# pavel-paulau/query

Hardware: AMD Instinct MI355X
Metric: rows/sec filter+group-by on 100M synthetic JSON docs; achieved HBM GB/s (higher is better)
Workload: dtype int64/f64 tagged scalars (u8 tag + 8 B payload), u32 dictionary codes; 1 GPU; config2: SELECT cat, SUM(price) FROM default WHERE price > 50 GROUP BY cat @ 100000000 rows, K_cat=1000, columns resident in HBM; rows_per_gpu=100000000, groups=1000, rows_selected=49401294, agg_mode=2, spec_kernel=1

## Files before the change

### query_amd/csrc/n1k_kernels.h

```cpp
#pragma once
#include <hip/hip_runtime.h>
#include <vector>
#include "n1k_types.h"

namespace n1k {

constexpr int kFilterStreamTile = 8192;

struct OutValue {
    uint64_t tag;
    uint64_t payload;
};

struct OutPartial {
    int64_t count;
    int64_t isum;
    double fsum;
    uint32_t flags;
    uint32_t ext_tag;
    uint64_t ext_payload;
    int64_t distinct;
};

struct SynthArgs {
    uint64_t seed, first_row, nrows, total_rows;
    uint32_t k_cat, pad;
    const double* cat_cdf;
    uint32_t* cat_codes;
    uint8_t* price_tags;
    uint64_t* price_payload;
    uint8_t* user_tags;
    uint64_t* user_payload;
    uint8_t* region_tags;
    uint64_t* region_payload;
};

hipError_t launch_init_table(const Program& P, const GlobalTable& G, uint64_t first, uint64_t count,
                             unsigned long long* counters, hipStream_t st);
hipError_t launch_restamp_ranks(const Program& P, const GlobalTable& G, hipStream_t st);
hipError_t launch_rehash(const Program& P, const GlobalTable& oldt, const GlobalTable& newt, uint32_t* err_flags,
                         unsigned long long* ngroups_scratch, hipStream_t st);
hipError_t launch_scan_group(const Program& P, const ScanArgs& A, const GlobalTable& G, unsigned long long* ngroups,
                             uint32_t grid, uint32_t block, uint32_t rows_per_lane, bool direct, hipStream_t st);
hipError_t launch_scan_fast(const Program& P, const FastArgs& F, const GlobalTable& G, unsigned long long* ngroups,
                            uint32_t grid, uint32_t block, uint32_t rows_per_lane, hipStream_t st);
hipError_t launch_merge_slabs(const Program& P, const FastArgs& F, const GlobalTable& G, uint32_t nblocks,
                              unsigned long long* ngroups, hipStream_t st, uint32_t ychunks_opt = 0);
hipError_t launch_finalize_region(const Program& P, const uint64_t* region, uint64_t cap, uint64_t count, OutValue* out_keys,
                                  OutValue* out_aggs, OutPartial* out_parts, uint64_t* out_rep, uint32_t* err_flags, hipStream_t st,
                                  const uint32_t* cand = nullptr, OutValue* ord = nullptr, bool ord_is_key = false, uint32_t ord_index = 0,
                                  uint64_t* images = nullptr, bool desc = false);
hipError_t launch_add_counter(unsigned long long* p, unsigned long long v, hipStream_t st);
hipError_t launch_probe_keys(const Program& P, uint64_t nrows, const GlobalTable& G, uint32_t* err_flags, unsigned long long* ngroups,
                             uint32_t grid, hipStream_t st);
hipError_t launch_project_records(const Program& P, const ProjectArgs& A, uint32_t grid, hipStream_t st);
hipError_t launch_agg_bins(const Program& P, const BinAggArgs& A, const GlobalTable& G, unsigned long long* ngroups, uint32_t grid,
                           hipStream_t st);
size_t topk_state_bytes();
size_t topk_ncand_offset();
hipError_t launch_topk_select(const Program& P, const OutValue* vals, uint32_t stride, uint32_t index, uint64_t n, bool desc,
                              uint64_t keep, uint64_t* images, void* state, uint32_t* cand, hipStream_t st, bool sampled = false, bool images_done = false);
bool topk_can_sample(uint64_t n, uint64_t keep);
uint64_t topk_cand_entries(uint64_t n);
hipError_t launch_topk_compact(const uint32_t* cand, uint64_t ncand, uint32_t nk, uint32_t na, const OutValue* keys,
                               const OutValue* aggs, const OutPartial* parts, const uint64_t* rep, OutValue* okeys, OutValue* oaggs,
                               OutPartial* oparts, uint64_t* orep, hipStream_t st);
hipError_t launch_distinct_layout(const Program& P, const GlobalTable& G, const DistinctArgs& D, hipStream_t st);
hipError_t launch_radix_pass(const RadixArgs& A, uint32_t slices, hipStream_t st, bool have_hist = false);
hipError_t launch_distinct_dedupe(const Program& P, const GlobalTable& G, const DedupeArgs& D, uint32_t grid, uint32_t block, hipStream_t st);
size_t distinct_dedupe_lds(const DedupeArgs& D);
hipError_t launch_compact_regions(const uint64_t* region, uint32_t nreg, uint64_t cap, const unsigned long long* count, const uint64_t* off,
                                  uint64_t* dst, hipStream_t st);
hipError_t launch_regrow_regions(const uint64_t* src, uint32_t nreg, uint64_t src_cap, uint64_t* dst, uint64_t dst_cap,
                                 unsigned long long* count, hipStream_t st);
hipError_t launch_distinct_words_global(const GlobalTable& G, const uint64_t* words, uint64_t n, uint64_t* table, uint64_t mask,
                                        uint32_t key_shift, unsigned long long* counts, uint32_t* err_flags, uint32_t grid,
                                        hipStream_t st);
hipError_t launch_distinct_add_counts(const Program& P, const GlobalTable& G, const unsigned long long* counts, uint32_t glob_off,
                                      hipStream_t st, const uint32_t* veto = nullptr);
hipError_t launch_distinct_insert(const Program& P, const GlobalTable& G, const DistinctArgs& D, uint32_t* err_flags,
                                  hipStream_t st);
hipError_t launch_export_partials(const Program& P, const GlobalTable& G, uint32_t nparts, uint64_t cap, uint64_t* out,
                                  uint64_t region_words, uint32_t* err_flags, hipStream_t st);
hipError_t launch_merge_partials(const Program& P, const GlobalTable& G, uint32_t nregions, uint64_t cap, const uint64_t* in,
                                 uint64_t region_words, uint32_t* err_flags, unsigned long long* ngroups, hipStream_t st,
                                 uint64_t limit = 0, bool unique_keys = false);
hipError_t launch_arith(const ArithArgs& A, hipStream_t st);
hipError_t launch_publish_counters(const unsigned long long* src, unsigned long long* dst, uint32_t n, hipStream_t st);
hipError_t launch_partition(const Program& P, const PartArgs& A, uint32_t grid, hipStream_t st);
struct HeaderList { unsigned long long* h[kMaxParts]; };
hipError_t launch_exchange_verdict(const HeaderList& H, uint32_t nregions, uint32_t* err_flags, hipStream_t st);
hipError_t launch_stamp_verdict(unsigned long long* headers, uint32_t nregions, uint64_t stride_words, const uint32_t* err_flags,
                                uint32_t host_status, hipStream_t st);
hipError_t launch_dense_to_segments(unsigned long long* headers, uint32_t nregions, uint64_t stride_words, uint64_t sub_rows, hipStream_t st,
                                    const uint32_t* dest_cap = nullptr);
struct SpecEntry {
    const char* name;
    SpecSig sig;
    hipError_t (*launch)(const Program& P, const FastArgs& F, const GlobalTable& G, unsigned long long* ngroups,
                         uint32_t grid, uint32_t block, bool wide, const WordLogArgs& L, hipStream_t st);
// ... 48 lines not shown
```

### query_amd/csrc/n1k_kernels.hip

```cpp
#include <hip/hip_runtime.h>
#include "n1k_device.h"
#include "n1k_tables.h"
#include "n1k_scatter.h"
#include "n1k_kernels.h"
#include <algorithm>
#include <vector>

namespace n1k {


template <int R>
N1K_DEV void load_operand(const Program& P, const Operand& o, const uint64_t (&row)[R], const bool (&valid)[R],
                          uint32_t (&tag)[R], uint64_t (&pay)[R]) {
    if (o.is_const) {
#pragma unroll
        for (int j = 0; j < R; j++) {
            tag[j] = o.ctag;
            pay[j] = o.cpayload;
        }
        return;
    }
    const DevCol& c = P.cols[o.col];
    if (c.kind == COLK_DICT32) {
        const uint32_t* codes = c.codes;
// ... 1235 lines not shown
            if (!pass[j]) continue;
            uint64_t r = s_base[dest[j]] + pos[j];
            if (r >= (A.per_dest ? (uint64_t)A.dest_cap[dest[j]] : A.capacity)) {
                if (!(atomicOr(A.err_flags, (uint32_t)ERR_TABLE_FULL) & ERR_TABLE_FULL) && A.region_bytes)
                    for (uint32_t q = 0; q < A.nparts; q++)
                        atomicOr(&A.counts[(size_t)q * A.count_stride + 1], 1ull);
                pass[j] = false;
            }
            pos[j] = A.region_bytes ? r : (uint64_t)dest[j] * A.capacity + r;
        }
        __syncthreads();
        for (uint32_t d = tid; d < A.nparts; d += BLOCK) s_cnt[d] = 0;
        uint64_t roff[R];
#pragma unroll
        for (int j = 0; j < R; j++) roff[j] = A.hdr_bytes;
        for (uint32_t c = 0; c < A.ncopy; c++) {
            Operand o{};
            o.is_const = 0;
            o.col = c;
            uint32_t vt[R];
            uint64_t vp[R];
            load_operand<R>(P, o, row, pass, vt, vp);
#pragma unroll
            for (int j = 0; j < R; j++) {
                if (!pass[j]) continue;
                if (A.per_dest) {
                    char* const reg = (char*)A.counts + (size_t)dest[j] * A.region_bytes;
                    const uint64_t capd = A.dest_cap[dest[j]];
                    if (P.cols[c].kind == COLK_DICT32) {
                        ((uint32_t*)(reg + roff[j]))[pos[j]] = (uint32_t)vp[j];
                        roff[j] = part_region_next(roff[j], capd, 4);
                    } else {
                        ((uint64_t*)(reg + roff[j]))[pos[j]] = vp[j];
                        roff[j] = part_region_next(roff[j], capd, 8);
                        ((uint8_t*)(reg + roff[j]))[pos[j]] = (uint8_t)vt[j];
                        roff[j] = part_region_next(roff[j], capd, 1);
                    }
                    continue;
                }
                const size_t shift = (size_t)dest[j] * A.region_bytes;
                if (P.cols[c].kind == COLK_DICT32) {
                    ((uint32_t*)((char*)A.out_codes[c] + shift))[pos[j]] = (uint32_t)vp[j];
                } else {
                    ((uint8_t*)((char*)A.out_tags[c] + shift))[pos[j]] = (uint8_t)vt[j];
                    ((uint64_t*)((char*)A.out_payload[c] + shift))[pos[j]] = vp[j];
                }
            }
        }
    }
    if (unsupported) atomicOr(A.err_flags, (uint32_t)ERR_UNSUPPORTED_VALUE);
    if (unpackable) atomicOr(A.err_flags, (uint32_t)ERR_UNPACKABLE_KEY);
}

enum { RED_ADD_U64, RED_ADD_F64, RED_OR, RED_MIN_I64, RED_MAX_I64, RED_MIN_U64, RED_MAX_U64 };

template <int OP>
N1K_DEV uint64_t reduce_over_y(uint64_t (*red)[64], uint64_t v) {
    const uint32_t tx = threadIdx.x, ty = threadIdx.y;
    red[ty][tx] = v;
    __syncthreads();
    for (uint32_t off = 8; off > 0; off >>= 1) {
        if (ty < off) {
            uint64_t a = red[ty][tx], b = red[ty + off][tx], r;
            if (OP == RED_ADD_U64) r = a + b;
            else if (OP == RED_ADD_F64) r = f64_bits(as_f64(a) + as_f64(b));
            else if (OP == RED_OR) r = a | b;
            else if (OP == RED_MIN_I64) r = (int64_t)a < (int64_t)b ? a : b;
            else if (OP == RED_MAX_I64) r = (int64_t)a > (int64_t)b ? a : b;
            else if (OP == RED_MIN_U64) r = a < b ? a : b;
            else r = a > b ? a : b;
            red[ty][tx] = r;
        }
        __syncthreads();
    }
    uint64_t out = red[0][tx];
    __syncthreads();
    return out;
}

__global__ __launch_bounds__(1024) void merge_slabs_kernel(const Program P, const FastArgs F, const GlobalTable G,
                                                          uint32_t nblocks_total, unsigned long long* ngroups) {
    __shared__ uint64_t red[16][64];
    const uint32_t S = F.lds_slots;
    const uint32_t s = blockIdx.x * 64 + threadIdx.x;
    const bool in_range = s < S;
    if (blockIdx.x == 0 && blockIdx.y == 0 && threadIdx.y == 0) {
        unsigned long long c = 0;
        for (uint32_t b = threadIdx.x; b < nblocks_total; b += 64) c += F.block_selected[b];
        for (int off = 32; off > 0; off >>= 1) c += __shfl_down(c, off, 64);
        if (threadIdx.x == 0 && c) atomicAdd(F.rows_selected, c);
    }
    const uint32_t Y = 16 * gridDim.y, y = blockIdx.y * 16 + threadIdx.y;
    const size_t slab_words = (size_t)P.lds_words * S * Y;
    const uint32_t nblocks = (in_range && y < nblocks_total) ? (nblocks_total - y + Y - 1) / Y : 0;
    const uint64_t* base = F.slabs + (size_t)y * P.lds_words * S + (in_range ? s : 0);
    uint64_t touched = 0;
#pragma unroll 8
    for (uint32_t b = 0; b < nblocks; b++) touched |= base[b * slab_words] ^ kEmptyKey;
    touched = reduce_over_y<RED_OR>(red, touched);
    const bool leader = threadIdx.y == 0 && in_range && touched != 0;
    long long g = -1;
    if (leader) g = global_find_or_insert(G, fast_slot_key(F, s), F.err_flags, ngroups);
    uint64_t* grow = g >= 0 ? &G.acc[(size_t)g * P.glob_words] : nullptr;
    for (uint32_t a = 0; a < P.naggs; a++) {
        const AggSpec& ag = P.aggs[a];
        if (ag.distinct) continue;
        const uint64_t* l = base + (size_t)ag.lds_off * S;
        unsigned long long* w = grow ? (unsigned long long*)(grow + ag.glob_off) : nullptr;
        switch (ag.kind) {
            case AGG_COUNT:
            case AGG_COUNTN: {
                unsigned long long c = 0;
#pragma unroll 8
                for (uint32_t b = 0; b < nblocks; b++) c += l[b * slab_words];
                c = reduce_over_y<RED_ADD_U64>(red, c);
                if (w && c) atomicAdd(&w[0], c);
                break;
            }
            case AGG_SUM:
            case AGG_AVG: {
                unsigned long long lo = 0, hi = 0, fl = 0, n = 0;
                double fs = 0.0;
                const bool avg = ag.kind == AGG_AVG;
#pragma unroll 4
                for (uint32_t b = 0; b < nblocks; b++) {
                    const uint64_t* lb = l + b * slab_words;
                    int64_t x = (int64_t)lb[0];
                    double f = as_f64(lb[(size_t)S]);
                    fl |= lb[2 * (size_t)S];
                    lo += (unsigned long long)(uint32_t)x;
                    hi += (unsigned long long)(x >> 32);
                    fs += f;
                    if (avg) n += lb[3 * (size_t)S];
                }
                lo = reduce_over_y<RED_ADD_U64>(red, lo);
                hi = reduce_over_y<RED_ADD_U64>(red, hi);
                fs = as_f64(reduce_over_y<RED_ADD_F64>(red, f64_bits(fs)));
                fl = reduce_over_y<RED_OR>(red, fl);
                if (avg) n = reduce_over_y<RED_ADD_U64>(red, n);
                if (!w || !fl) break;
                if (fl & (SF_NONNEG_INT | SF_NEG_INT)) { atomicAdd(&w[0], lo); atomicAdd(&w[1], hi); }
                if (fl & SF_FLOAT) atomicAdd((double*)&w[2], fs);
                atomicOr(&w[3], fl);
                if (avg) atomicAdd(&w[4], n);
                break;
            }
            default: {
                const bool mn = ag.kind == AGG_MIN;
                unsigned long long fl = 0;
                long long iv = mn ? INT64_MAX : INT64_MIN;
                unsigned long long fv = mn ? ~0ull : 0ull, sv = mn ? ~0ull : 0ull;
#pragma unroll 4
                for (uint32_t b = 0; b < nblocks; b++) {
                    const uint64_t* lb = l + b * slab_words;
                    fl |= lb[0];
                    long long x = (long long)lb[(size_t)S];
                    unsigned long long yv = lb[2 * (size_t)S], z = lb[3 * (size_t)S];
                    iv = mn ? (x < iv ? x : iv) : (x > iv ? x : iv);
                    fv = mn ? (yv < fv ? yv : fv) : (yv > fv ? yv : fv);
                    sv = mn ? (z < sv ? z : sv) : (z > sv ? z : sv);
                }
                fl = reduce_over_y<RED_OR>(red, fl);
                if (mn) {
                    iv = (long long)reduce_over_y<RED_MIN_I64>(red, (uint64_t)iv);
                    fv = reduce_over_y<RED_MIN_U64>(red, fv);
                    sv = reduce_over_y<RED_MIN_U64>(red, sv);
                } else {
                    iv = (long long)reduce_over_y<RED_MAX_I64>(red, (uint64_t)iv);
                    fv = reduce_over_y<RED_MAX_U64>(red, fv);
                    sv = reduce_over_y<RED_MAX_U64>(red, sv);
                }
                if (!w || !fl) break;
                atomicOr(&w[0], fl);
                if (fl & MM_INT) { if (mn) atomicMin((long long*)&w[1], iv); else atomicMax((long long*)&w[1], iv); }
                if (fl & MM_FLOAT) { if (mn) atomicMin(&w[2], fv); else atomicMax(&w[2], fv); }
                if (fl & MM_STRING) { if (mn) atomicMin(&w[3], sv); else atomicMax(&w[3], sv); }
                break;
            }
        }
    }
}

__global__ void export_partials_kernel(const Program P, const GlobalTable G, uint32_t nparts, uint64_t cap,
                                       uint64_t* out, uint64_t region_words, uint32_t* err_flags) {
    uint64_t s = (uint64_t)blockIdx.x * blockDim.x + threadIdx.x;
    if (s == 0 && P.wide_count && *P.wide_count)
        for (uint32_t r = 0; r < nparts; r++) atomicOr((unsigned long long*)&out[(size_t)r * region_words + 1], 2ull);
    const uint64_t key = s < G.capacity ? G.keys[s] : kEmptyKey;
    const bool used = key != kEmptyKey;
    const uint32_t d = used ? (uint32_t)(((mix64(key) >> 32) * (uint64_t)nparts) >> 32) : 0xFFFFFFFFu;
    unsigned long long pos = 0;
    unsigned long long todo = __ballot(used);
    const uint32_t lane = threadIdx.x & 63;
    while (todo) {
        const int leader = __ffsll((long long)todo) - 1;
        const uint32_t dl = __shfl(d, leader, 64);
        const unsigned long long same = __ballot(used && d == dl);
        unsigned long long base = 0;
        if ((int)lane == leader) base = atomicAdd((unsigned long long*)&out[(size_t)dl * region_words], (unsigned long long)__popcll(same));
        base = __shfl(base, leader, 64);
        if (used && d == dl) pos = base + (unsigned long long)__popcll(same & ((1ull << lane) - 1ull));
        todo &= ~same;
    }
    if (!used) return;
    uint64_t* region = out + (size_t)d * region_words;
    if (pos >= cap) {
        if (!(atomicOr(err_flags, (uint32_t)ERR_TABLE_FULL) & ERR_TABLE_FULL))
            for (uint32_t r = 0; r < nparts; r++) atomicOr((unsigned long long*)&out[(size_t)r * region_words + 1], 1ull);
        return;
    }
    region[2 + pos] = key;
    uint64_t* acc = region + 2 + cap + pos * P.glob_words;
    for (uint32_t w = 0; w < P.glob_words; w++) acc[w] = G.acc[(size_t)s * P.glob_words + w];
}

N1K_DEV void merge_partial_record(const Program& P, const GlobalTable& G, uint64_t key, const uint64_t* l, uint32_t* err_flags,
                                  bool& fresh, bool unique_keys) {
    long long g = global_find_or_insert_quiet(G, key, err_flags, fresh);
    if (g < 0) return;
    if (fresh && unique_keys) {
        uint64_t* w = &G.acc[(size_t)g * P.glob_words];
        for (uint32_t i = 0; i < P.glob_words; i++) w[i] = l[i];
        return;
    }
    for (uint32_t a = 0; a < P.naggs; a++) {
        const AggSpec& ag = P.aggs[a];
        const uint64_t* p = l + ag.glob_off;
        unsigned long long* w = (unsigned long long*)&G.acc[(size_t)g * P.glob_words + ag.glob_off];
        if (ag.distinct) {
            atomicOr(err_flags, (uint32_t)ERR_UNSUPPORTED_VALUE);
            continue;
// ... 1160 lines not shown
    hipLaunchKernelGGL(rehash_kernel, dim3(blocks), dim3(256), 0, st, P, oldt, newt, err_flags, ngroups_scratch);
    return hipGetLastError();
}

template <int R, int BLOCK>
static hipError_t launch_scan_variant(const Program& P, const ScanArgs& A, const GlobalTable& G, unsigned long long* ngroups,
                                      uint32_t grid, bool direct, size_t shmem, hipStream_t st) {
    if (direct) {
        auto k = scan_group_kernel<R, BLOCK, true>;
        if (shmem > 48 * 1024) (void)hipFuncSetAttribute((const void*)k, hipFuncAttributeMaxDynamicSharedMemorySize, (int)shmem);
        hipLaunchKernelGGL(k, dim3(grid), dim3(BLOCK), shmem, st, P, A, G, ngroups);
    } else {
        auto k = scan_group_kernel<R, BLOCK, false>;
        if (shmem > 48 * 1024) (void)hipFuncSetAttribute((const void*)k, hipFuncAttributeMaxDynamicSharedMemorySize, (int)shmem);
        hipLaunchKernelGGL(k, dim3(grid), dim3(BLOCK), shmem, st, P, A, G, ngroups);
    }
    return hipGetLastError();
}

hipError_t launch_scan_group(const Program& P, const ScanArgs& A, const GlobalTable& G, unsigned long long* ngroups,
                             uint32_t grid, uint32_t block, uint32_t rows_per_lane, bool direct, hipStream_t st) {
    size_t shmem = (size_t)A.lds_slots * P.lds_words * 8 + (size_t)A.dcache_slots * A.dcache_aggs * 8;
    if (block == 256) return launch_scan_variant<4, 256>(P, A, G, ngroups, grid, direct, shmem, st);
    if (block == 512) return launch_scan_variant<4, 512>(P, A, G, ngroups, grid, direct, shmem, st);
    if (rows_per_lane == 2) return launch_scan_variant<2, 1024>(P, A, G, ngroups, grid, direct, shmem, st);
    return launch_scan_variant<4, 1024>(P, A, G, ngroups, grid, direct, shmem, st);
}

template <int R, int BLOCK>
static hipError_t launch_fast_variant(const Program& P, const FastArgs& F, const GlobalTable& G, unsigned long long* ngroups,
                                      uint32_t grid, size_t shmem, hipStream_t st) {
    auto k = scan_fast_kernel<R, BLOCK>;
    if (shmem > 48 * 1024) (void)hipFuncSetAttribute((const void*)k, hipFuncAttributeMaxDynamicSharedMemorySize, (int)shmem);
    hipLaunchKernelGGL(k, dim3(grid), dim3(BLOCK), shmem, st, P, F, G, ngroups);
    return hipGetLastError();
}

hipError_t launch_scan_fast(const Program& P, const FastArgs& F, const GlobalTable& G, unsigned long long* ngroups,
                            uint32_t grid, uint32_t block, uint32_t rows_per_lane, hipStream_t st) {
    size_t shmem = (size_t)F.lds_slots * P.lds_words * 8;
    for (uint32_t t = 0; t < F.nterms; t++)
        if (term_is_table_bit(F.terms[t].op) && F.terms[t].match_n <= kMatchLdsBytes) {
            shmem += kMatchLdsBytes;
            break;
        }
    if (block == 512) {
        if (rows_per_lane == 2) return launch_fast_variant<2, 512>(P, F, G, ngroups, grid, shmem, st);
        return launch_fast_variant<4, 512>(P, F, G, ngroups, grid, shmem, st);
    }
    if (rows_per_lane == 2) return launch_fast_variant<2, 1024>(P, F, G, ngroups, grid, shmem, st);
    return launch_fast_variant<4, 1024>(P, F, G, ngroups, grid, shmem, st);
}

hipError_t launch_merge_slabs(const Program& P, const FastArgs& F, const GlobalTable& G, uint32_t nblocks,
                              unsigned long long* ngroups, hipStream_t st, uint32_t ychunks_opt) {
    uint32_t blocks = (F.lds_slots + 63) / 64;
    uint32_t ychunks = nblocks >= 512 ? 4 : (nblocks >= 128 ? 2 : 1);
    while (ychunks < 16 && blocks * ychunks < 256 && nblocks >= 32 * ychunks) ychunks *= 2;
    if (ychunks_opt) ychunks = ychunks_opt;
    hipLaunchKernelGGL(merge_slabs_kernel, dim3(blocks, ychunks), dim3(64, 16), 0, st, P, F, G, nblocks, ngroups);
    return hipGetLastError();
}

__global__ void add_counter_kernel(unsigned long long* p, unsigned long long v) { *p += v; }

hipError_t launch_add_counter(unsigned long long* p, unsigned long long v, hipStream_t st) {
    hipLaunchKernelGGL(add_counter_kernel, dim3(1), dim3(1), 0, st, p, v);
    return hipGetLastError();
}

hipError_t launch_finalize_region(const Program& P, const uint64_t* region, uint64_t cap, uint64_t count, OutValue* out_keys,
                                  OutValue* out_aggs, OutPartial* out_parts, uint64_t* out_rep, uint32_t* err_flags, hipStream_t st,
                                  const uint32_t* cand, OutValue* ord, bool ord_is_key, uint32_t ord_index, uint64_t* images, bool desc) {
    if (!count) return hipSuccess;
    hipLaunchKernelGGL(finalize_region_kernel, dim3((uint32_t)((count + 255) / 256)), dim3(256), 0, st, P, region, cap, count,
                       out_keys, out_aggs, out_parts, out_rep, err_flags, cand, ord, ord_is_key ? 1u : 0u, ord_index, images, desc ? 1u : 0u);
    return hipGetLastError();
}

hipError_t launch_probe_keys(const Program& P, uint64_t nrows, const GlobalTable& G, uint32_t* err_flags, unsigned long long* ngroups,
                             uint32_t grid, hipStream_t st) {
    hipLaunchKernelGGL((probe_keys_kernel<4, 256>), dim3(grid), dim3(256), 0, st, P, nrows, G, err_flags, ngroups);
    return hipGetLastError();
}

hipError_t launch_project_records(const Program& P, const ProjectArgs& A, uint32_t grid, hipStream_t st) {
    hipLaunchKernelGGL((project_records_kernel<4, 512>), dim3(grid), dim3(512), 0, st, P, A);
    return hipGetLastError();
}

hipError_t launch_agg_bins(const Program& P, const BinAggArgs& A, const GlobalTable& G, unsigned long long* ngroups, uint32_t grid,
                           hipStream_t st) {
    auto k = agg_bins_kernel<512>;
    size_t shmem = (size_t)A.lds_slots * P.lds_words * 8;
    if (shmem > 48 * 1024) (void)hipFuncSetAttribute((const void*)k, hipFuncAttributeMaxDynamicSharedMemorySize, (int)shmem);
    hipLaunchKernelGGL(k, dim3(grid), dim3(512), shmem, st, P, A, G, ngroups);
    return hipGetLastError();
}

size_t topk_state_bytes() { return sizeof(TopkState); }

uint64_t topk_cand_entries(uint64_t n) { return n + (uint64_t)kTopkSegs * (n / kTopkSegs + 320); }
bool topk_can_sample(uint64_t n, uint64_t keep) { return n >= 4ull * kTopkSample && n < (1ull << 32) && keep * 2 * kTopkSample / n + 16 <= kTopkSample / 4; }

hipError_t launch_topk_select(const Program& P, const OutValue* vals, uint32_t stride, uint32_t index, uint64_t n, bool desc,
                              uint64_t keep, uint64_t* images, void* state, uint32_t* cand, hipStream_t st, bool sampled,
                              bool images_done) {
    TopkState* S = (TopkState*)state;
    (void)hipMemsetAsync(S, 0, sizeof(TopkState), st);
    const uint32_t blocks = (uint32_t)((n + 255) / 256);
    if (!images_done)
        hipLaunchKernelGGL(topk_images_kernel, dim3(blocks), dim3(256), 0, st, P, vals, stride, index, n, desc ? 1u : 0u, images, S, keep);
    else
        hipLaunchKernelGGL(topk_state_kernel, dim3(1), dim3(1), 0, st, S, keep);
// ... 254 lines not shown
```

Baseline: 321.8 billion rows/s.

## Rewrite slab merge as op-table driven batched kernel with LDS-atomic reduction

Replaces the per-aggregate merge kernel, which used repeated shared-memory tree reductions across y, with a templated kernel. It encodes each LDS word's fold op in a table and loads batches of slabs across several words at once, optionally as 16-byte vector loads covering two slots. Partial results are combined through LDS atomics instead of log-step syncthreads reductions, and the grid is resized so lanes can be split across multiple slab rows. The aim is to cut synchronisation and serial reduction overhead in the merge phase, at the cost of many template variants, more register pressure and a changed argument meaning for the row override.

```diff
diff --git a/query_amd/csrc/n1k_kernels.h b/query_amd/csrc/n1k_kernels.h
--- a/query_amd/csrc/n1k_kernels.h
+++ b/query_amd/csrc/n1k_kernels.h
@@ -44,8 +44,8 @@
                              uint32_t grid, uint32_t block, uint32_t rows_per_lane, bool direct, hipStream_t st);
 hipError_t launch_scan_fast(const Program& P, const FastArgs& F, const GlobalTable& G, unsigned long long* ngroups,
                             uint32_t grid, uint32_t block, uint32_t rows_per_lane, hipStream_t st);
-hipError_t launch_merge_slabs(const Program& P, const FastArgs& F, const GlobalTable& G, uint32_t nblocks,
-                              unsigned long long* ngroups, hipStream_t st, uint32_t ychunks_opt = 0);
+hipError_t launch_merge_slabs(const Program& P, const FastArgs& F, const GlobalTable& G, uint32_t nslabs,
+                              unsigned long long* ngroups, hipStream_t st, uint32_t rows_opt = 0);
 hipError_t launch_finalize_region(const Program& P, const uint64_t* region, uint64_t cap, uint64_t count, OutValue* out_keys,
                                   OutValue* out_aggs, OutPartial* out_parts, uint64_t* out_rep, uint32_t* err_flags, hipStream_t st,
                                   const uint32_t* cand = nullptr, OutValue* ord = nullptr, bool ord_is_key = false, uint32_t ord_index = 0,
diff --git a/query_amd/csrc/n1k_kernels.hip b/query_amd/csrc/n1k_kernels.hip
--- a/query_amd/csrc/n1k_kernels.hip
+++ b/query_amd/csrc/n1k_kernels.hip
@@ -1311,131 +1311,178 @@
     if (unpackable) atomicOr(A.err_flags, (uint32_t)ERR_UNPACKABLE_KEY);
 }
 
-enum { RED_ADD_U64, RED_ADD_F64, RED_OR, RED_MIN_I64, RED_MAX_I64, RED_MIN_U64, RED_MAX_U64 };
-
-template <int OP>
-N1K_DEV uint64_t reduce_over_y(uint64_t (*red)[64], uint64_t v) {
-    const uint32_t tx = threadIdx.x, ty = threadIdx.y;
-    red[ty][tx] = v;
-    __syncthreads();
-    for (uint32_t off = 8; off > 0; off >>= 1) {
-        if (ty < off) {
-            uint64_t a = red[ty][tx], b = red[ty + off][tx], r;
-            if (OP == RED_ADD_U64) r = a + b;
-            else if (OP == RED_ADD_F64) r = f64_bits(as_f64(a) + as_f64(b));
-            else if (OP == RED_OR) r = a | b;
-            else if (OP == RED_MIN_I64) r = (int64_t)a < (int64_t)b ? a : b;
-            else if (OP == RED_MAX_I64) r = (int64_t)a > (int64_t)b ? a : b;
-            else if (OP == RED_MIN_U64) r = a < b ? a : b;
-            else r = a > b ? a : b;
-            red[ty][tx] = r;
+enum : uint8_t { MOP_NONE, MOP_TOUCH, MOP_ADD, MOP_SUMI, MOP_SUMF, MOP_OR, MOP_MINI, MOP_MAXI, MOP_MINU, MOP_MAXU };
+
+struct MergeOps {
+    uint8_t op[kMaxLdsWords];
+    uint16_t goff[kMaxLdsWords];
+};
+
+constexpr int merge_batch(int W) { return 12 / W > 8 ? 8 : (12 / W < 1 ? 1 : 12 / W); }
+
+N1K_DEV uint64_t merge_ident(uint32_t op) {
+    return op == MOP_MINI ? (uint64_t)INT64_MAX : (op == MOP_MAXI ? (uint64_t)INT64_MIN : (op == MOP_MINU ? ~0ull : 0ull));
+}
+
+N1K_DEV void merge_fold(uint32_t op, uint64_t& a, uint64_t& h, uint64_t x) {
+    switch (op) {
+        case MOP_TOUCH: a |= x ^ kEmptyKey; break;
+        case MOP_ADD: a += x; break;
+        case MOP_SUMI: a += (uint64_t)(uint32_t)x; h += (uint64_t)((int64_t)x >> 32); break;
+        case MOP_SUMF: a = f64_bits(as_f64(a) + as_f64(x)); break;
+        case MOP_OR: a |= x; break;
+        case MOP_MINI: a = (int64_t)x < (int64_t)a ? x : a; break;
+        case MOP_MAXI: a = (int64_t)x > (int64_t)a ? x : a; break;
+        case MOP_MINU: a = x < a ? x : a; break;
+        case MOP_MAXU: a = x > a ? x : a; break;
+        default: break;
+    }
+}
+
+template <uint32_t OP, int B, int V>
+N1K_DEV void merge_fold_batch(uint64_t (&a)[V], uint64_t (&h)[V], const uint64_t (&d)[B][V], const bool (&valid)[B]) {
+#pragma unroll
+    for (int j = 0; j < B; j++) {
+        if (!valid[j]) continue;
+#pragma unroll
+        for (int v = 0; v < V; v++) merge_fold(OP, a[v], h[v], d[j][v]);
+    }
+}
+
+template <int B, int V>
+N1K_DEV void merge_fold_word(uint32_t op, uint64_t (&a)[V], uint64_t (&h)[V], const uint64_t (&d)[B][V], const bool (&valid)[B]) {
+    switch (op) {
+        case MOP_TOUCH: merge_fold_batch<MOP_TOUCH>(a, h, d, valid); break;
+        case MOP_ADD: merge_fold_batch<MOP_ADD>(a, h, d, valid); break;
+        case MOP_SUMI: merge_fold_batch<MOP_SUMI>(a, h, d, valid); break;
+        case MOP_SUMF: merge_fold_batch<MOP_SUMF>(a, h, d, valid); break;
+        case MOP_OR: merge_fold_batch<MOP_OR>(a, h, d, valid); break;
+        case MOP_MINI: merge_fold_batch<MOP_MINI>(a, h, d, valid); break;
+        case MOP_MAXI: merge_fold_batch<MOP_MAXI>(a, h, d, valid); break;
+        case MOP_MINU: merge_fold_batch<MOP_MINU>(a, h, d, valid); break;
+        case MOP_MAXU: merge_fold_batch<MOP_MAXU>(a, h, d, valid); break;
+        default: break;
+    }
+}
+
+template <int V>
+N1K_DEV void merge_fold_lds(uint32_t op, lds_u64* p, lds_u64* ph, const uint64_t (&a)[V], const uint64_t (&h)[V]) {
+#define N1K_EACH_SLOT(stmt) for (int v = 0; v < V; v++) { stmt; } break
+    switch (op) {
+        case MOP_TOUCH:
+        case MOP_OR: N1K_EACH_SLOT(lds_or_u64(p + v, a[v]));
+        case MOP_ADD: N1K_EACH_SLOT(lds_add_u64(p + v, a[v]));
+        case MOP_SUMI: N1K_EACH_SLOT(lds_add_u64(p + v, a[v]); lds_add_u64(ph + v, h[v]));
+        case MOP_SUMF: N1K_EACH_SLOT(lds_add_f64(p + v, as_f64(a[v])));
+        case MOP_MINI: N1K_EACH_SLOT(lds_min_i64(p + v, (long long)a[v]));
+        case MOP_MAXI: N1K_EACH_SLOT(lds_max_i64(p + v, (long long)a[v]));
+        case MOP_MINU: N1K_EACH_SLOT(lds_min_u64(p + v, a[v]));
+        case MOP_MAXU: N1K_EACH_SLOT(lds_max_u64(p + v, a[v]));
+        default: break;
+    }
+#undef N1K_EACH_SLOT
+}
+
+N1K_DEV void merge_apply(uint32_t op, unsigned long long* w, uint64_t a, uint64_t h) {
+    switch (op) {
+        case MOP_ADD: if (a) atomicAdd(w, (unsigned long long)a); break;
+        case MOP_SUMI: if (a | h) { atomicAdd(&w[0], (unsigned long long)a); atomicAdd(&w[1], (unsigned long long)h); } break;
+        case MOP_SUMF: if (a) atomicAdd((double*)w, as_f64(a)); break;
+        case MOP_OR: if (a) atomicOr(w, (unsigned long long)a); break;
+        case MOP_MINI: if ((int64_t)a != INT64_MAX) atomicMin((long long*)w, (long long)a); break;
+        case MOP_MAXI: if ((int64_t)a != INT64_MIN) atomicMax((long long*)w, (long long)a); break;
+        case MOP_MINU: if (a != ~0ull) atomicMin(w, (unsigned long long)a); break;
+        case MOP_MAXU: if (a) atomicMax(w, (unsigned long long)a); break;
+        default: break;
+    }
+}
+
+template <int W, int V, bool LOOPED>
+__global__ __launch_bounds__(1024) void merge_slabs_kernel(const Program P, const FastArgs F, const GlobalTable G, const MergeOps M,
+                                                          uint32_t nslabs, unsigned long long* ngroups, uint32_t sub_shift) {
+    constexpr int B = merge_batch(W);
+    __shared__ uint64_t red[2 * W][64 * V];
+    const uint32_t S = F.lds_slots, LW = P.lds_words;
+    const uint32_t lane = threadIdx.x, ty = __builtin_amdgcn_readfirstlane(threadIdx.y);
+    const uint32_t SL = 64u >> sub_shift, slane = lane & (SL - 1);
+    const uint32_t brows = blockDim.y << sub_shift, brow = (ty << sub_shift) + (lane >> (6 - sub_shift));
+    const uint32_t s = (blockIdx.x * SL + slane) * V;
+    const bool in_range = s < S;
+    const uint32_t rows = brows * gridDim.y, r = blockIdx.y * brows + brow;
+    const size_t slab_words = (size_t)LW * S;
+    const uint32_t lane_off = (in_range ? s : 0u) * 8u;
+    bool count_rows = blockIdx.x == 0 && blockIdx.y == 0 && ty == 0;
+    __shared__ long long grp[64 * V];
+    for (uint32_t w0 = 0; w0 < (LOOPED ? LW : 1u); w0 += W) {
+        uint32_t op[W];
+        uint64_t acc[W][V], hi[W][V];
+#pragma unroll
+        for (int k = 0; k < W; k++) {
+            op[k] = w0 + k < LW ? (uint32_t)M.op[w0 + k] : (uint32_t)MOP_NONE;
+#pragma unroll
+            for (int v = 0; v < V; v++) {
+                acc[k][v] = merge_ident(op[k]);
+                hi[k][v] = 0;
+            }
+        }
+        for (uint64_t b0 = r;; b0 += (uint64_t)B * rows) {
+            uint64_t d[W][B][V];
+            bool valid[B];
+#pragma unroll
+            for (int j = 0; j < B; j++) {
+                const uint64_t b = b0 + (uint64_t)j * rows;
+                valid[j] = b < nslabs;
+                const uint64_t* sl = F.slabs + (size_t)(valid[j] ? b : 0ull) * slab_words;
+#pragma unroll
+                for (int k = 0; k < W; k++) {
+                    const uint32_t w = w0 + k < LW ? w0 + k : LW - 1;
+                    if constexpr (V == 2) {
+                        const ulonglong2 q = *(const ulonglong2*)((const char*)(sl + (size_t)w * S) + lane_off);
+                        d[k][j][0] = q.x;
+                        d[k][j][1] = q.y;
+                    } else {
+                        d[k][j][0] = *(const uint64_t*)((const char*)(sl + (size_t)w * S) + lane_off);
+                    }
+                }
+            }
+            if (count_rows) {
+                unsigned long long c = 0;
+                for (uint32_t i = lane; i < nslabs; i += 64) c += F.block_selected[i];
+                for (int off = 32; off > 0; off >>= 1) c += __shfl_down(c, off, 64);
+                if (lane == 0 && c) atomicAdd(F.rows_selected, c);
+                count_rows = false;
+            }
+#pragma unroll
+            for (int k = 0; k < W; k++) merge_fold_word<B, V>(op[k], acc[k], hi[k], d[k], valid);
+            if (!LOOPED || b0 + (uint64_t)B * rows >= nslabs) break;
+        }
+        if (LOOPED && w0) __syncthreads();
+        if (brow == 0) {
+#pragma unroll
+            for (int k = 0; k < W; k++)
+#pragma unroll
+                for (int v = 0; v < V; v++) {
+                    red[k][slane * V + v] = acc[k][v];
+                    red[W + k][slane * V + v] = hi[k][v];
+                }
         }
         __syncthreads();
-    }
-    uint64_t out = red[0][tx];
-    __syncthreads();
-    return out;
-}
-
-__global__ __launch_bounds__(1024) void merge_slabs_kernel(const Program P, const FastArgs F, const GlobalTable G,
-                                                          uint32_t nblocks_total, unsigned long long* ngroups) {
-    __shared__ uint64_t red[16][64];
-    const uint32_t S = F.lds_slots;
-    const uint32_t s = blockIdx.x * 64 + threadIdx.x;
-    const bool in_range = s < S;
-    if (blockIdx.x == 0 && blockIdx.y == 0 && threadIdx.y == 0) {
-        unsigned long long c = 0;
-        for (uint32_t b = threadIdx.x; b < nblocks_total; b += 64) c += F.block_selected[b];
-        for (int off = 32; off > 0; off >>= 1) c += __shfl_down(c, off, 64);
-        if (threadIdx.x == 0 && c) atomicAdd(F.rows_selected, c);
-    }
-    const uint32_t Y = 16 * gridDim.y, y = blockIdx.y * 16 + threadIdx.y;
-    const size_t slab_words = (size_t)P.lds_words * S * Y;
-    const uint32_t nblocks = (in_range && y < nblocks_total) ? (nblocks_total - y + Y - 1) / Y : 0;
-    const uint64_t* base = F.slabs + (size_t)y * P.lds_words * S + (in_range ? s : 0);
-    uint64_t touched = 0;
-#pragma unroll 8
-    for (uint32_t b = 0; b < nblocks; b++) touched |= base[b * slab_words] ^ kEmptyKey;
-    touched = reduce_over_y<RED_OR>(red, touched);
-    const bool leader = threadIdx.y == 0 && in_range && touched != 0;
-    long long g = -1;
-    if (leader) g = global_find_or_insert(G, fast_slot_key(F, s), F.err_flags, ngroups);
-    uint64_t* grow = g >= 0 ? &G.acc[(size_t)g * P.glob_words] : nullptr;
-    for (uint32_t a = 0; a < P.naggs; a++) {
-        const AggSpec& ag = P.aggs[a];
-        if (ag.distinct) continue;
-        const uint64_t* l = base + (size_t)ag.lds_off * S;
-        unsigned long long* w = grow ? (unsigned long long*)(grow + ag.glob_off) : nullptr;
-        switch (ag.kind) {
-            case AGG_COUNT:
-            case AGG_COUNTN: {
-                unsigned long long c = 0;
-#pragma unroll 8
-                for (uint32_t b = 0; b < nblocks; b++) c += l[b * slab_words];
-                c = reduce_over_y<RED_ADD_U64>(red, c);
-                if (w && c) atomicAdd(&w[0], c);
-                break;
-            }
-            case AGG_SUM:
-            case AGG_AVG: {
-                unsigned long long lo = 0, hi = 0, fl = 0, n = 0;
-                double fs = 0.0;
-                const bool avg = ag.kind == AGG_AVG;
-#pragma unroll 4
-                for (uint32_t b = 0; b < nblocks; b++) {
-                    const uint64_t* lb = l + b * slab_words;
-                    int64_t x = (int64_t)lb[0];
-                    double f = as_f64(lb[(size_t)S]);
-                    fl |= lb[2 * (size_t)S];
-                    lo += (unsigned long long)(uint32_t)x;
-                    hi += (unsigned long long)(x >> 32);
-                    fs += f;
-                    if (avg) n += lb[3 * (size_t)S];
-                }
-                lo = reduce_over_y<RED_ADD_U64>(red, lo);
-                hi = reduce_over_y<RED_ADD_U64>(red, hi);
-                fs = as_f64(reduce_over_y<RED_ADD_F64>(red, f64_bits(fs)));
-                fl = reduce_over_y<RED_OR>(red, fl);
-                if (avg) n = reduce_over_y<RED_ADD_U64>(red, n);
-                if (!w || !fl) break;
-                if (fl & (SF_NONNEG_INT | SF_NEG_INT)) { atomicAdd(&w[0], lo); atomicAdd(&w[1], hi); }
-                if (fl & SF_FLOAT) atomicAdd((double*)&w[2], fs);
-                atomicOr(&w[3], fl);
-                if (avg) atomicAdd(&w[4], n);
-                break;
-            }
-            default: {
-                const bool mn = ag.kind == AGG_MIN;
-                unsigned long long fl = 0;
-                long long iv = mn ? INT64_MAX : INT64_MIN;
-                unsigned long long fv = mn ? ~0ull : 0ull, sv = mn ? ~0ull : 0ull;
-#pragma unroll 4
-                for (uint32_t b = 0; b < nblocks; b++) {
-                    const uint64_t* lb = l + b * slab_words;
-                    fl |= lb[0];
-                    long long x = (long long)lb[(size_t)S];
-                    unsigned long long yv = lb[2 * (size_t)S], z = lb[3 * (size_t)S];
-                    iv = mn ? (x < iv ? x : iv) : (x > iv ? x : iv);
-                    fv = mn ? (yv < fv ? yv : fv) : (yv > fv ? yv : fv);
-                    sv = mn ? (z < sv ? z : sv) : (z > sv ? z : sv);
-                }
-                fl = reduce_over_y<RED_OR>(red, fl);
-                if (mn) {
-                    iv = (long long)reduce_over_y<RED_MIN_I64>(red, (uint64_t)iv);
-                    fv = reduce_over_y<RED_MIN_U64>(red, fv);
-                    sv = reduce_over_y<RED_MIN_U64>(red, sv);
-                } else {
-                    iv = (long long)reduce_over_y<RED_MAX_I64>(red, (uint64_t)iv);
-                    fv = reduce_over_y<RED_MAX_U64>(red, fv);
-                    sv = reduce_over_y<RED_MAX_U64>(red, sv);
-                }
-                if (!w || !fl) break;
-                atomicOr(&w[0], fl);
-                if (fl & MM_INT) { if (mn) atomicMin((long long*)&w[1], iv); else atomicMax((long long*)&w[1], iv); }
-                if (fl & MM_FLOAT) { if (mn) atomicMin(&w[2], fv); else atomicMax(&w[2], fv); }
-                if (fl & MM_STRING) { if (mn) atomicMin(&w[3], sv); else atomicMax(&w[3], sv); }
-                break;
-            }
+        if (brow != 0) {
+#pragma unroll
+            for (int k = 0; k < W; k++) merge_fold_lds<V>(op[k], lds_word(&red[k][0], slane * V), lds_word(&red[W + k][0], slane * V), acc[k], hi[k]);
+        }
+        __syncthreads();
+        for (uint32_t v = brow; v < (in_range ? (uint32_t)V : 0u); v += brows) {
+            const uint32_t e = slane * V + v;
+            long long g = -1;
+            if (w0 != 0) g = grp[e];
+            else if (red[0][e] != 0) g = global_find_or_insert(G, fast_slot_key(F, s + v), F.err_flags, ngroups);
+            if (LOOPED && w0 == 0) grp[e] = g;
+            if (g < 0) continue;
+            uint64_t* const grow = &G.acc[(size_t)g * P.glob_words];
+#pragma unroll
+            for (int k = 0; k < W; k++)
+                if (w0 + k < LW) merge_apply(op[k], (unsigned long long*)(grow + M.goff[w0 + k]), red[k][e], red[W + k][e]);
         }
     }
 }
@@ -2702,14 +2749,74 @@
     return launch_fast_variant<4, 1024>(P, F, G, ngroups, grid, shmem, st);
 }
 
-hipError_t launch_merge_slabs(const Program& P, const FastArgs& F, const GlobalTable& G, uint32_t nblocks,
-                              unsigned long long* ngroups, hipStream_t st, uint32_t ychunks_opt) {
-    uint32_t blocks = (F.lds_slots + 63) / 64;
-    uint32_t ychunks = nblocks >= 512 ? 4 : (nblocks >= 128 ? 2 : 1);
-    while (ychunks < 16 && blocks * ychunks < 256 && nblocks >= 32 * ychunks) ychunks *= 2;
-    if (ychunks_opt) ychunks = ychunks_opt;
-    hipLaunchKernelGGL(merge_slabs_kernel, dim3(blocks, ychunks), dim3(64, 16), 0, st, P, F, G, nblocks, ngroups);
-    return hipGetLastError();
+template <int W, int V, bool LOOPED>
+static hipError_t launch_merge_variant(const Program& P, const FastArgs& F, const GlobalTable& G, const MergeOps& M, uint32_t nslabs,
+                                       unsigned long long* ngroups, dim3 grid, dim3 block, uint32_t sub_shift, hipStream_t st) {
+    hipLaunchKernelGGL((merge_slabs_kernel<W, V, LOOPED>), grid, block, 0, st, P, F, G, M, nslabs, ngroups, sub_shift);
+    return hipGetLastError();
+}
+
+template <int V>
+static hipError_t launch_merge_width(const Program& P, const FastArgs& F, const GlobalTable& G, const MergeOps& M, uint32_t nslabs,
+                                     unsigned long long* ngroups, hipStream_t st, uint32_t rows_opt) {
+    const uint32_t W = P.lds_words;
+    const bool known = W == 2 || W == 4 || W == 5 || W == 9;
+    const uint32_t B = (uint32_t)merge_batch(known ? (int)W : 4);
+    const uint32_t rows_needed = (nslabs + B - 1) / B;
+    uint32_t sub_shift = 0;
+    while (sub_shift < (V == 2 ? 3u : 2u) && (2u << sub_shift) <= rows_needed) sub_shift++;
+    const uint32_t sub = 1u << sub_shift, slots_x = (64u >> sub_shift) * V;
+    const uint32_t xblocks = (F.lds_slots + slots_x - 1) / slots_x;
+    uint32_t gy = (rows_needed + 16 * sub - 1) / (16 * sub);
+    while (gy < 4 && xblocks * gy < 256 && (gy + 1) * sub <= rows_needed) gy++;
+    uint32_t ty = (rows_needed + gy * sub - 1) / (gy * sub);
+    if (rows_opt) {
+        ty = 16;
+        gy = rows_opt;
+    }
+    const dim3 grid(xblocks, gy), block(64, ty);
+    if (!known || (uint64_t)B * ty * sub * gy < nslabs) return launch_merge_variant<4, V, true>(P, F, G, M, nslabs, ngroups, grid, block, sub_shift, st);
+    if (W == 2) return launch_merge_variant<2, V, false>(P, F, G, M, nslabs, ngroups, grid, block, sub_shift, st);
+    if (W == 4) return launch_merge_variant<4, V, false>(P, F, G, M, nslabs, ngroups, grid, block, sub_shift, st);
+    if (W == 5) return launch_merge_variant<5, V, false>(P, F, G, M, nslabs, ngroups, grid, block, sub_shift, st);
+    return launch_merge_variant<9, V, false>(P, F, G, M, nslabs, ngroups, grid, block, sub_shift, st);
+}
+
+hipError_t launch_merge_slabs(const Program& P, const FastArgs& F, const GlobalTable& G, uint32_t nslabs,
+                              unsigned long long* ngroups, hipStream_t st, uint32_t rows_opt) {
+    MergeOps M;
+    for (int i = 0; i < kMaxLdsWords; i++) {
+        M.op[i] = MOP_NONE;
+        M.goff[i] = 0;
+    }
+    M.op[0] = MOP_TOUCH;
+    for (uint32_t a = 0; a < P.naggs; a++) {
+        const AggSpec& ag = P.aggs[a];
+        if (ag.distinct) continue;
+        uint8_t* op = &M.op[ag.lds_off];
+        uint16_t* go = &M.goff[ag.lds_off];
+        switch (ag.kind) {
+            case AGG_COUNT:
+            case AGG_COUNTN:
+                op[0] = MOP_ADD, go[0] = (uint16_t)ag.glob_off;
+                break;
+            case AGG_SUM:
+            case AGG_AVG:
+                op[0] = MOP_SUMI, go[0] = (uint16_t)ag.glob_off;
+                op[1] = MOP_SUMF, go[1] = (uint16_t)(ag.glob_off + 2);
+                op[2] = MOP_OR, go[2] = (uint16_t)(ag.glob_off + 3);
+                if (ag.kind == AGG_AVG) op[3] = MOP_ADD, go[3] = (uint16_t)(ag.glob_off + 4);
+                break;
+            default: {
+                const bool mn = ag.kind == AGG_MIN;
+                op[0] = MOP_OR, op[1] = mn ? MOP_MINI : MOP_MAXI, op[2] = op[3] = mn ? MOP_MINU : MOP_MAXU;
+                for (int i = 0; i < 4; i++) go[i] = (uint16_t)(ag.glob_off + i);
+                break;
+            }
+        }
+    }
+    if (F.lds_slots % 2 == 0 && (uintptr_t)F.slabs % 16 == 0) return launch_merge_width<2>(P, F, G, M, nslabs, ngroups, st, rows_opt);
+    return launch_merge_width<1>(P, F, G, M, nslabs, ngroups, st, rows_opt);
 }
 
 __global__ void add_counter_kernel(unsigned long long* p, unsigned long long v) { *p += v; }
```

Result: no change. 321.3 billion rows/s (-0.2%).

## Restructure slab merge: per-block slot groups, per-word reductions, fast home-slot insert

Applied to the files above, without the earlier changes.

Rewrites the merge-slabs kernel so each 1024-thread block owns 8 slots, with 128 lanes per slot striding over the per-block slabs. Slab words are handled generically by a per-word op table, loads are batched six at a time, and partials are reduced by wave shuffles and then a single LDS pass across waves. This replaces the repeated __syncthreads tree reductions and the old 2D grid. The global-table insert first tries a CAS on the hash home slot before falling back to the probing insert. The aim is to raise memory-level parallelism and cut sync overhead in the merge phase, at the cost of reading every slab word even for unused aggregate layouts and of larger dynamic LDS.

```diff
diff --git a/query_amd/csrc/n1k_kernels.hip b/query_amd/csrc/n1k_kernels.hip
--- a/query_amd/csrc/n1k_kernels.hip
+++ b/query_amd/csrc/n1k_kernels.hip
@@ -1311,129 +1311,221 @@
     if (unpackable) atomicOr(A.err_flags, (uint32_t)ERR_UNPACKABLE_KEY);
 }
 
-enum { RED_ADD_U64, RED_ADD_F64, RED_OR, RED_MIN_I64, RED_MAX_I64, RED_MIN_U64, RED_MAX_U64 };
-
-template <int OP>
-N1K_DEV uint64_t reduce_over_y(uint64_t (*red)[64], uint64_t v) {
-    const uint32_t tx = threadIdx.x, ty = threadIdx.y;
-    red[ty][tx] = v;
-    __syncthreads();
-    for (uint32_t off = 8; off > 0; off >>= 1) {
-        if (ty < off) {
-            uint64_t a = red[ty][tx], b = red[ty + off][tx], r;
-            if (OP == RED_ADD_U64) r = a + b;
-            else if (OP == RED_ADD_F64) r = f64_bits(as_f64(a) + as_f64(b));
-            else if (OP == RED_OR) r = a | b;
-            else if (OP == RED_MIN_I64) r = (int64_t)a < (int64_t)b ? a : b;
-            else if (OP == RED_MAX_I64) r = (int64_t)a > (int64_t)b ? a : b;
-            else if (OP == RED_MIN_U64) r = a < b ? a : b;
-            else r = a > b ? a : b;
-            red[ty][tx] = r;
-        }
-        __syncthreads();
-    }
-    uint64_t out = red[0][tx];
-    __syncthreads();
-    return out;
-}
-
-__global__ __launch_bounds__(1024) void merge_slabs_kernel(const Program P, const FastArgs F, const GlobalTable G,
-                                                          uint32_t nblocks_total, unsigned long long* ngroups) {
-    __shared__ uint64_t red[16][64];
-    const uint32_t S = F.lds_slots;
-    const uint32_t s = blockIdx.x * 64 + threadIdx.x;
-    const bool in_range = s < S;
-    if (blockIdx.x == 0 && blockIdx.y == 0 && threadIdx.y == 0) {
-        unsigned long long c = 0;
-        for (uint32_t b = threadIdx.x; b < nblocks_total; b += 64) c += F.block_selected[b];
-        for (int off = 32; off > 0; off >>= 1) c += __shfl_down(c, off, 64);
-        if (threadIdx.x == 0 && c) atomicAdd(F.rows_selected, c);
-    }
-    const uint32_t Y = 16 * gridDim.y, y = blockIdx.y * 16 + threadIdx.y;
-    const size_t slab_words = (size_t)P.lds_words * S * Y;
-    const uint32_t nblocks = (in_range && y < nblocks_total) ? (nblocks_total - y + Y - 1) / Y : 0;
-    const uint64_t* base = F.slabs + (size_t)y * P.lds_words * S + (in_range ? s : 0);
-    uint64_t touched = 0;
-#pragma unroll 8
-    for (uint32_t b = 0; b < nblocks; b++) touched |= base[b * slab_words] ^ kEmptyKey;
-    touched = reduce_over_y<RED_OR>(red, touched);
-    const bool leader = threadIdx.y == 0 && in_range && touched != 0;
-    long long g = -1;
-    if (leader) g = global_find_or_insert(G, fast_slot_key(F, s), F.err_flags, ngroups);
-    uint64_t* grow = g >= 0 ? &G.acc[(size_t)g * P.glob_words] : nullptr;
+enum : uint32_t { MW_SKIP = 0, MW_TOUCH, MW_ADD, MW_ISUM, MW_FADD, MW_OR, MW_MIN_I64, MW_MAX_I64, MW_MIN_U64, MW_MAX_U64 };
+
+#ifndef N1K_MERGE_SLOTS
+#define N1K_MERGE_SLOTS 8
+#endif
+constexpr int kMergeSlots = N1K_MERGE_SLOTS, kMergeBlock = 1024, kMergeWaves = kMergeBlock / 64;
+constexpr int kMergeLanes = kMergeBlock / kMergeSlots;
+constexpr int kMergeWords = 4, kMergeSlabs = 6;
+static_assert(64 % kMergeSlots == 0 && kMergeSlots >= 8, "a wave holds whole slot ranges; a slab word of a range is >= 64 bytes");
+
+N1K_DEV uint32_t merge_word_op(const Program& P, uint32_t w, uint32_t& agg) {
+    agg = 0;
+    if (w == 0) return MW_TOUCH;
+    if (w >= P.lds_words) return MW_SKIP;
+    for (uint32_t a = 0; a < P.naggs; a++) {
+        const AggSpec& ag = P.aggs[a];
+        if (ag.distinct || w < ag.lds_off) continue;
+        const uint32_t i = w - ag.lds_off;
+        agg = a;
+        switch (ag.kind) {
+            case AGG_COUNT:
+            case AGG_COUNTN:
+                if (i == 0) return MW_ADD;
+                break;
+            case AGG_SUM:
+            case AGG_AVG:
+                if (i == 0) return MW_ISUM;
+                if (i == 1) return MW_FADD;
+                if (i == 2) return MW_OR;
+                if (i == 3 && ag.kind == AGG_AVG) return MW_ADD;
+                break;
+            default:
+                if (i == 0) return MW_OR;
+                if (i == 1) return ag.kind == AGG_MIN ? MW_MIN_I64 : MW_MAX_I64;
+                if (i < kWordsMinMax) return ag.kind == AGG_MIN ? MW_MIN_U64 : MW_MAX_U64;
+                break;
+        }
+    }
+    return MW_SKIP;
+}
+
+N1K_DEV uint64_t merge_word_identity(uint32_t op) {
+    return op == MW_MIN_I64 ? (uint64_t)INT64_MAX : (op == MW_MAX_I64 ? (uint64_t)INT64_MIN : (op == MW_MIN_U64 ? ~0ull : 0ull));
+}
+
+N1K_DEV uint64_t merge_word_combine(uint32_t op, uint64_t a, uint64_t b) {
+    switch (op) {
+        case MW_FADD: return f64_bits(as_f64(a) + as_f64(b));
+        case MW_TOUCH:
+        case MW_OR: return a | b;
+        case MW_MIN_I64: return (int64_t)b < (int64_t)a ? b : a;
+        case MW_MAX_I64: return (int64_t)b > (int64_t)a ? b : a;
+        case MW_MIN_U64: return b < a ? b : a;
+        case MW_MAX_U64: return b > a ? b : a;
+        default: return a + b;
+    }
+}
+
+N1K_DEV long long merge_insert_key(const GlobalTable& G, uint64_t key, uint64_t home, unsigned long long seen, uint32_t* err_flags,
+                                   unsigned long long* ngroups) {
+    if (seen == key) return (long long)home;
+    if (seen == kEmptyKey) {
+        unsigned long long old = atomicCAS((unsigned long long*)&G.keys[home], (unsigned long long)kEmptyKey, (unsigned long long)key);
+        if (old == kEmptyKey) {
+            const unsigned long long active = __ballot(1);
+            if (__builtin_amdgcn_mbcnt_hi((uint32_t)(active >> 32), __builtin_amdgcn_mbcnt_lo((uint32_t)active, 0u)) == 0u)
+                atomicAdd(ngroups, (unsigned long long)__popcll(active));
+            return (long long)home;
+        }
+        if (old == key) return (long long)home;
+    }
+    return global_find_or_insert(G, key, err_flags, ngroups);
+}
+
+__global__ __launch_bounds__(kMergeBlock) void merge_slabs_kernel(const Program P, const FastArgs F, const GlobalTable G,
+                                                                  uint32_t nblocks_total, uint32_t ways,
+                                                                  unsigned long long* ngroups) {
+    extern __shared__ uint64_t red[];
+    constexpr int R = kMergeSlots, U = kMergeSlabs, WP = kMergeWords;
+    const uint32_t S = F.lds_slots, W = P.lds_words, nvals = W + P.naggs;
+    const uint32_t tid = threadIdx.x, r = tid % R, lane = tid / R, wave = tid / 64;
+    const uint32_t s = blockIdx.x * R + r;
+    const bool slot_ok = s < S;
+    const bool lane_ok = slot_ok && lane < ways;
+    const uint32_t per_lane = (nblocks_total + ways - 1) / ways;
+    const uint64_t* const base = F.slabs + (slot_ok ? s : 0u);
+    const size_t slab_words = (size_t)W * S;
+    const uint64_t key = fast_slot_key(F, slot_ok ? s : 0u);
+    const uint64_t home = mix64(key) & (G.capacity - 1);
+    const unsigned long long seen = __hip_atomic_load((unsigned long long*)&G.keys[home], __ATOMIC_RELAXED, __HIP_MEMORY_SCOPE_AGENT);
+    unsigned long long sel = 0;
+    if (blockIdx.x == 0)
+        for (uint32_t b0 = 0; b0 < nblocks_total; b0 += kMergeBlock) {
+            const uint32_t b = b0 + tid;
+            const unsigned long long x = F.block_selected[b < nblocks_total ? b : 0u];
+            sel += b < nblocks_total ? x : 0ull;
+        }
+
+    for (uint32_t w0 = 0; w0 < W; w0 += WP) {
+        uint32_t op[WP], agg[WP];
+        uint64_t acc[WP], acc_hi[WP];
+        size_t woff[WP];
+#pragma unroll
+        for (int i = 0; i < WP; i++) {
+            op[i] = merge_word_op(P, w0 + i, agg[i]);
+            acc[i] = merge_word_identity(op[i]);
+            acc_hi[i] = 0;
+            woff[i] = (size_t)(w0 + i < W ? w0 + i : 0u) * S;
+        }
+        for (uint32_t b0 = 0; b0 < per_lane; b0 += U) {
+            uint64_t v[WP][U];
+            bool m[U];
+            size_t boff[U];
+#pragma unroll
+            for (int j = 0; j < U; j++) {
+                const uint32_t b = lane + (b0 + j) * ways;
+                m[j] = lane_ok && b0 + j < per_lane && b < nblocks_total;
+                boff[j] = (size_t)(m[j] ? b : 0u) * slab_words;
+            }
+#pragma unroll
+            for (int i = 0; i < WP; i++)
+#pragma unroll
+                for (int j = 0; j < U; j++) v[i][j] = base[boff[j] + woff[i]];
+#pragma unroll
+            for (int i = 0; i < WP; i++) {
+                if (op[i] == MW_SKIP) continue;
+                if (op[i] == MW_TOUCH) {
+#pragma unroll
+                    for (int j = 0; j < U; j++) acc[i] |= m[j] ? v[i][j] ^ kEmptyKey : 0ull;
+                } else if (op[i] == MW_ISUM) {
+#pragma unroll
+                    for (int j = 0; j < U; j++) {
+                        const int64_t x = m[j] ? (int64_t)v[i][j] : 0;
+                        acc[i] += (uint64_t)(uint32_t)x;
+                        acc_hi[i] += (uint64_t)(x >> 32);
+                    }
+                } else {
+#pragma unroll
+                    for (int j = 0; j < U; j++) acc[i] = m[j] ? merge_word_combine(op[i], acc[i], v[i][j]) : acc[i];
+                }
+            }
+        }
+#pragma unroll
+        for (int i = 0; i < WP; i++) {
+            if (op[i] == MW_SKIP) continue;
+            for (int off = R; off < 64; off <<= 1) {
+                acc[i] = merge_word_combine(op[i], acc[i], __shfl_xor(acc[i], off, 64));
+                if (op[i] == MW_ISUM) acc_hi[i] += __shfl_xor(acc_hi[i], off, 64);
+            }
+            if ((tid & 63u) < (uint32_t)R) {
+                red[((size_t)wave * nvals + w0 + i) * R + r] = acc[i];
+                if (op[i] == MW_ISUM) red[((size_t)wave * nvals + W + agg[i]) * R + r] = acc_hi[i];
+            }
+        }
+    }
+    __syncthreads();
+
+    if (blockIdx.x == 0) {
+        for (int off = 32; off > 0; off >>= 1) sel += __shfl_down(sel, off, 64);
+        if ((tid & 63u) == 0 && sel) atomicAdd(F.rows_selected, sel);
+    }
+    if (tid >= (uint32_t)R || !slot_ok) return;
+
+    auto over_waves = [&](uint32_t op, uint32_t v) {
+        uint64_t x = red[(size_t)v * R + r];
+#pragma unroll
+        for (int wv = 1; wv < kMergeWaves; wv++) x = merge_word_combine(op, x, red[((size_t)wv * nvals + v) * R + r]);
+        return x;
+    };
+    if (!over_waves(MW_OR, 0)) return;
+    const long long g = merge_insert_key(G, key, home, seen, F.err_flags, ngroups);
+    if (g < 0) return;
+    uint64_t* const grow = &G.acc[(size_t)g * P.glob_words];
     for (uint32_t a = 0; a < P.naggs; a++) {
         const AggSpec& ag = P.aggs[a];
         if (ag.distinct) continue;
-        const uint64_t* l = base + (size_t)ag.lds_off * S;
-        unsigned long long* w = grow ? (unsigned long long*)(grow + ag.glob_off) : nullptr;
+        const uint32_t l = ag.lds_off;
+        unsigned long long* w = (unsigned long long*)(grow + ag.glob_off);
         switch (ag.kind) {
             case AGG_COUNT:
             case AGG_COUNTN: {
-                unsigned long long c = 0;
-#pragma unroll 8
-                for (uint32_t b = 0; b < nblocks; b++) c += l[b * slab_words];
-                c = reduce_over_y<RED_ADD_U64>(red, c);
-                if (w && c) atomicAdd(&w[0], c);
+                const unsigned long long c = over_waves(MW_ADD, l);
+                if (c) atomicAdd(&w[0], c);
                 break;
             }
             case AGG_SUM:
             case AGG_AVG: {
-                unsigned long long lo = 0, hi = 0, fl = 0, n = 0;
-                double fs = 0.0;
-                const bool avg = ag.kind == AGG_AVG;
-#pragma unroll 4
-                for (uint32_t b = 0; b < nblocks; b++) {
-                    const uint64_t* lb = l + b * slab_words;
-                    int64_t x = (int64_t)lb[0];
-                    double f = as_f64(lb[(size_t)S]);
-                    fl |= lb[2 * (size_t)S];
-                    lo += (unsigned long long)(uint32_t)x;
-                    hi += (unsigned long long)(x >> 32);
-                    fs += f;
-                    if (avg) n += lb[3 * (size_t)S];
-                }
-                lo = reduce_over_y<RED_ADD_U64>(red, lo);
-                hi = reduce_over_y<RED_ADD_U64>(red, hi);
-                fs = as_f64(reduce_over_y<RED_ADD_F64>(red, f64_bits(fs)));
-                fl = reduce_over_y<RED_OR>(red, fl);
-                if (avg) n = reduce_over_y<RED_ADD_U64>(red, n);
-                if (!w || !fl) break;
-                if (fl & (SF_NONNEG_INT | SF_NEG_INT)) { atomicAdd(&w[0], lo); atomicAdd(&w[1], hi); }
-                if (fl & SF_FLOAT) atomicAdd((double*)&w[2], fs);
+                const unsigned long long fl = over_waves(MW_OR, l + 2);
+                if (!fl) break;
+                if (fl & (SF_NONNEG_INT | SF_NEG_INT)) {
+                    atomicAdd(&w[0], (unsigned long long)over_waves(MW_ADD, l));
+                    atomicAdd(&w[1], (unsigned long long)over_waves(MW_ADD, W + a));
+                }
+                if (fl & SF_FLOAT) atomicAdd((double*)&w[2], as_f64(over_waves(MW_FADD, l + 1)));
                 atomicOr(&w[3], fl);
-                if (avg) atomicAdd(&w[4], n);
+                if (ag.kind == AGG_AVG) atomicAdd(&w[4], (unsigned long long)over_waves(MW_ADD, l + 3));
                 break;
             }
             default: {
                 const bool mn = ag.kind == AGG_MIN;
-                unsigned long long fl = 0;
-                long long iv = mn ? INT64_MAX : INT64_MIN;
-                unsigned long long fv = mn ? ~0ull : 0ull, sv = mn ? ~0ull : 0ull;
-#pragma unroll 4
-                for (uint32_t b = 0; b < nblocks; b++) {
-                    const uint64_t* lb = l + b * slab_words;
-                    fl |= lb[0];
-                    long long x = (long long)lb[(size_t)S];
-                    unsigned long long yv = lb[2 * (size_t)S], z = lb[3 * (size_t)S];
-                    iv = mn ? (x < iv ? x : iv) : (x > iv ? x : iv);
-                    fv = mn ? (yv < fv ? yv : fv) : (yv > fv ? yv : fv);
-                    sv = mn ? (z < sv ? z : sv) : (z > sv ? z : sv);
-                }
-                fl = reduce_over_y<RED_OR>(red, fl);
-                if (mn) {
-                    iv = (long long)reduce_over_y<RED_MIN_I64>(red, (uint64_t)iv);
-                    fv = reduce_over_y<RED_MIN_U64>(red, fv);
-                    sv = reduce_over_y<RED_MIN_U64>(red, sv);
-                } else {
-                    iv = (long long)reduce_over_y<RED_MAX_I64>(red, (uint64_t)iv);
-                    fv = reduce_over_y<RED_MAX_U64>(red, fv);
-                    sv = reduce_over_y<RED_MAX_U64>(red, sv);
-                }
-                if (!w || !fl) break;
+                const unsigned long long fl = over_waves(MW_OR, l);
+                if (!fl) break;
                 atomicOr(&w[0], fl);
-                if (fl & MM_INT) { if (mn) atomicMin((long long*)&w[1], iv); else atomicMax((long long*)&w[1], iv); }
-                if (fl & MM_FLOAT) { if (mn) atomicMin(&w[2], fv); else atomicMax(&w[2], fv); }
-                if (fl & MM_STRING) { if (mn) atomicMin(&w[3], sv); else atomicMax(&w[3], sv); }
+                if (fl & MM_INT) {
+                    const long long iv = (long long)over_waves(mn ? MW_MIN_I64 : MW_MAX_I64, l + 1);
+                    if (mn) atomicMin((long long*)&w[1], iv); else atomicMax((long long*)&w[1], iv);
+                }
+                if (fl & MM_FLOAT) {
+                    const unsigned long long fv = over_waves(mn ? MW_MIN_U64 : MW_MAX_U64, l + 2);
+                    if (mn) atomicMin(&w[2], fv); else atomicMax(&w[2], fv);
+                }
+                if (fl & MM_STRING) {
+                    const unsigned long long sv = over_waves(mn ? MW_MIN_U64 : MW_MAX_U64, l + 3);
+                    if (mn) atomicMin(&w[3], sv); else atomicMax(&w[3], sv);
+                }
                 break;
             }
         }
@@ -2704,11 +2796,12 @@
 
 hipError_t launch_merge_slabs(const Program& P, const FastArgs& F, const GlobalTable& G, uint32_t nblocks,
                               unsigned long long* ngroups, hipStream_t st, uint32_t ychunks_opt) {
-    uint32_t blocks = (F.lds_slots + 63) / 64;
-    uint32_t ychunks = nblocks >= 512 ? 4 : (nblocks >= 128 ? 2 : 1);
-    while (ychunks < 16 && blocks * ychunks < 256 && nblocks >= 32 * ychunks) ychunks *= 2;
-    if (ychunks_opt) ychunks = ychunks_opt;
-    hipLaunchKernelGGL(merge_slabs_kernel, dim3(blocks, ychunks), dim3(64, 16), 0, st, P, F, G, nblocks, ngroups);
+    const uint32_t blocks = (F.lds_slots + kMergeSlots - 1) / kMergeSlots;
+    const uint32_t ways = ychunks_opt ? std::min<uint32_t>(ychunks_opt, kMergeLanes) : (uint32_t)kMergeLanes;
+    const size_t shmem = (size_t)kMergeWaves * (P.lds_words + P.naggs) * kMergeSlots * 8;
+    if (shmem > 48 * 1024)
+        (void)hipFuncSetAttribute((const void*)merge_slabs_kernel, hipFuncAttributeMaxDynamicSharedMemorySize, (int)shmem);
+    hipLaunchKernelGGL(merge_slabs_kernel, dim3(blocks), dim3(kMergeBlock), shmem, st, P, F, G, nblocks, ways, ngroups);
     return hipGetLastError();
 }
 
```

Result: no change. 331.4 billion rows/s before, 331.0 billion rows/s after (median of 2 runs) (-0.1%).
